# miuda-ai/lele

Hardware: AMD Instinct MI355X
Metric: STFT+mel GB/s (SenseVoice front-end: PCM -> log-mel -> LFR, algorithmic bytes); SenseVoiceSmall-shaped RTF in `sensevoice` (higher is better)
Workload: dtype f32

## Files before the change

lele_amd/csrc/igemm_rs.h:

```cpp
#pragma once

namespace {

struct RsArgs {
    const int8_t* af;
    const int8_t* wf;
    unsigned rows;
    int n;
    int nrt, nct;
    int ncb, nrr;
    int8_t* hid;
    const float* x;
    const float* partial;
    int nblk;
    unsigned* hpart;
    unsigned* sync;
    unsigned* deverr;
#ifdef LELE_HIP_LAB
    long long* dbg;
    int ablate;
#endif
};
#ifdef LELE_HIP_LAB
#define RS_STAMP(who) do { if (g.dbg && lane == 0 && nstamp < 32 && wave < 9) g.dbg[((size_t)blockIdx.x * 9 + wave) * 32 + nstamp++] = (long long)wall_clock64(); } while (0)
// ... 695 lines not shown
        row = row < rows ? row : rows - 1u;
        r.scale = 1.0f;
        r.zp_i = epi.zp_a_fixed;
        if (epi.prm) {
            const unsigned sl = single ? 0u : row / mu;
            r.scale = epi.prm[sl].scale;
            r.zp_i = epi.prm[sl].zp_i;
        }
    };
    auto compute = [&](const v4i (&a)[KW], const Row& r, int t, int buf) {
        const unsigned row = (unsigned)t * 32u + (unsigned)l31;
        const bool rok = row < rows;
        const size_t at = (size_t)(rok ? row : rows - 1u) * (unsigned)n + (unsigned)(cok ? col : n - 4);
        float4 res1, res2;
        if (NRES > 0) res1 = *reinterpret_cast<const float4*>(epi.res1 + at);
        if (NRES > 1) res2 = *reinterpret_cast<const float4*>(epi.res2 + at);
        v16i acc;
#pragma unroll
        for (int i = 0; i < 16; ++i) acc[i] = 0;
        int rsp = 0;
#pragma unroll
        for (int s = 0; s < KW; ++s) {
            acc = __builtin_amdgcn_mfma_i32_32x32x32_i8(bf[s], a[s], acc, 0, 0, 0);
            rsp = __builtin_amdgcn_sdot4(a[s][0], 0x01010101, rsp, false);
            rsp = __builtin_amdgcn_sdot4(a[s][1], 0x01010101, rsp, false);
            rsp = __builtin_amdgcn_sdot4(a[s][2], 0x01010101, rsp, false);
            rsp = __builtin_amdgcn_sdot4(a[s][3], 0x01010101, rsp, false);
        }
#pragma unroll
        for (int gq = 0; gq < 4; ++gq) s_x[buf][wave][gq][lane] = v4i{acc[4 * gq], acc[4 * gq + 1], acc[4 * gq + 2], acc[4 * gq + 3]};
        s_rs[buf][wave][lane] = rsp;
        __syncthreads();
        v4i tot = s_x[buf][0][wave][lane];
        int rowsum = s_rs[buf][0][l31] + s_rs[buf][0][l31 + 32];
#pragma unroll
        for (int w = 1; w < 4; ++w) {
            const v4i p = s_x[buf][w][wave][lane];
            tot[0] += p[0], tot[1] += p[1], tot[2] += p[2], tot[3] += p[3];
            rowsum += s_rs[buf][w][l31] + s_rs[buf][w][l31 + 32];
        }
        const int ca = 128 - r.zp_i;
        const int rterm = cbz * rowsum + epi.k * ca * cbz;
        float4 o;
        o.x = rs_value(tot[0], rterm, ca, colsum[0], r.scale * ws[0], bias[0], has_ws, has_bias, epi.relu);
        o.y = rs_value(tot[1], rterm, ca, colsum[1], r.scale * ws[1], bias[1], has_ws, has_bias, epi.relu);
        o.z = rs_value(tot[2], rterm, ca, colsum[2], r.scale * ws[2], bias[2], has_ws, has_bias, epi.relu);
        o.w = rs_value(tot[3], rterm, ca, colsum[3], r.scale * ws[3], bias[3], has_ws, has_bias, epi.relu);
        if (NRES > 0) o.x = o.x + res1.x, o.y = o.y + res1.y, o.z = o.z + res1.z, o.w = o.w + res1.w;
        if (NRES > 1) o.x = o.x + res2.x, o.y = o.y + res2.y, o.z = o.z + res2.z, o.w = o.w + res2.w;
        if (rok && cok) *reinterpret_cast<float4*>(epi.out + at) = o;
    };
    v4i a0[KW], a1[KW];
    Row r0, r1;
    load_tile(a0, r0, t0);
    int t = t0;
    while (t + 1 < t1) {
        load_tile(a1, r1, t + 1);
        compute(a0, r0, t, 0);
        load_tile(a0, r0, t + 2 < t1 ? t + 2 : t1 - 1);
        compute(a1, r1, t + 1, 1);
        t += 2;
    }
    if (t < t1) compute(a0, r0, t, 0);
}

struct AsArgs {
    const float* x;
    const int8_t* wf;
    unsigned rows;
    int n, nct;
    const float* partial;
    int nblk;
    QParams* prm;
    int tpw;
    const float* ln_g = nullptr;
    const float* ln_b = nullptr;
    float ln_eps = 0.0f;
    float* ln_out = nullptr;
    float* ln_rowstat = nullptr;
    const float* fs_x = nullptr;
    int fs_pitch = 0;
    const float* fs_w = nullptr;
    const float* fs_b = nullptr;
};
constexpr int AS_LN_PITCH = 516;
constexpr int AS_LN_LDS = 32 * AS_LN_PITCH * 4;
constexpr int as_fs_lds(int fs) { return (32 + fs - 1) * AS_LN_PITCH * 4; }

__device__ __forceinline__ void as_ln_rows(const float* s_ln, const float* s_lng, const float* s_lnb, unsigned t, int wave, int hv, int l31,
                                           unsigned rows, float eps, float* ln_out, float* ln_rowstat) {
    constexpr int NT = 16;
    const float inv_n = 1.0f / 512.0f;
#pragma unroll
    for (int rr = 0; rr < 2; ++rr) {
        const int r = 2 * wave + hv + 16 * rr;
        const unsigned grow = t * 32u + (unsigned)r;
        float v[NT];
#pragma unroll
        for (int c = 0; c < NT; ++c) v[c] = s_ln[r * AS_LN_PITCH + 32 * c + l31];
        float sum, sumsq;
        row_sums_reg<NT, true, true>(v, 512, l31, &sum, &sumsq);
        const float mean = sum * inv_n;
        const float var = sumsq * inv_n - mean * mean;
        const float inv_std = 1.0f / sqrtf(var + eps);
        float mn = 3.40282347e+38f, mx = -3.40282347e+38f;
        float* orow = ln_out + (size_t)(grow < rows ? grow : rows - 1u) * 512u;
#pragma unroll
        for (int c = 0; c < NT; ++c) {
            const float tv = (v[c] - mean) * inv_std;
            const float o = fmaf_(tv, s_lng[32 * c + l31], s_lnb[32 * c + l31]);
            if (grow < rows) orow[32 * c + l31] = o;
            mn = o < mn ? o : mn;
            mx = o > mx ? o : mx;
        }
        if (ln_rowstat) {
            mn = group_allreduce32(mn, [](float cur, float a) { return a < cur ? a : cur; });
            mx = group_allreduce32(mx, [](float cur, float a) { return a > cur ? a : cur; });
            if (l31 == 0 && grow < rows) {
                ln_rowstat[2 * (size_t)grow] = mn;
                ln_rowstat[2 * (size_t)grow + 1] = mx;
            }
        }
    }
}

template <int NRES, bool RELU, bool TWO = true, bool LN = false, int FS = 0>
__global__ __launch_bounds__(512) void igemm_as_kernel(AsArgs g, IgemmEpi epi) {
    static_assert(!LN || TWO, "the LayerNorm needs whole rows in one workgroup");
    static_assert(FS == 0 || (LN && NRES >= 1), "the in-kernel FSMN block is res1 of the LayerNorm form");
    constexpr int KS = 16;
    extern __shared__ __attribute__((aligned(16))) float s_ln[];
    __shared__ float s_lng[LN ? 512 : 1], s_lnb[LN ? 512 : 1];
    __shared__ __attribute__((aligned(16))) char s_tile[KS * 1024];
    __shared__ int s_rowsum[4][32];
    __shared__ float s_scale[32];
    __shared__ int s_zp[32];
    __shared__ __attribute__((aligned(16))) int s_colsum[512];
    __shared__ __attribute__((aligned(16))) float s_ws[512];
    __shared__ __attribute__((aligned(16))) float s_bias[512];
    const int lane = threadIdx.x & 63, wave = __builtin_amdgcn_readfirstlane(threadIdx.x >> 6);
    const int hv = lane >> 5, l31 = lane & 31;
    const int t = blockIdx.x, n = g.n;
    const unsigned rows = g.rows, mu = (unsigned)epi.m;
    const int u = wave >> 2, kq = wave & 3, q4 = lane & 3, rsub = lane >> 2;
    const unsigned row_q = (unsigned)t * 32u + 16u * (unsigned)u + (unsigned)rsub;
    const unsigned rowc_q = row_q < rows ? row_q : rows - 1u;
    const unsigned first = (unsigned)t * 32u + 16u * (unsigned)u;
    const unsigned last = first + 15u < rows ? first + 15u : rows - 1u;
    const unsigned s_lo = (first < rows ? first : rows - 1u) / mu, s_hi = last / mu;
    float2 pw[2][4];
#pragma unroll
    for (int a = 0; a < 2; ++a) {
        const unsigned sl = s_lo + (unsigned)a < s_hi ? s_lo + (unsigned)a : s_hi;
        const float2* pp = reinterpret_cast<const float2*>(g.partial) + (size_t)sl * g.nblk;
#pragma unroll
        for (int j = 0; j < 4; ++j) {
            const int idx = lane + 64 * j;
            pw[a][j] = pp[idx < g.nblk ? idx : g.nblk - 1];
        }
    }
    float4 xv[8];
    {
        const float* src = g.x + (size_t)rowc_q * 512u + 128u * (unsigned)kq + 4u * (unsigned)q4;
#pragma unroll
        for (int c = 0; c < 8; ++c) xv[c] = *reinterpret_cast<const float4*>(src + 16 * c);
    }
    float fw[FS > 0 ? FS : 1], fbv = 0.0f;
    if constexpr (FS > 0) {
        const unsigned tile_base = (unsigned)(uintptr_t)(__attribute__((address_space(3))) float*)s_ln;
#pragma unroll
        for (int k2 = 0; k2 < (2 * (32 + FS - 1) + 7) / 8; ++k2) {
            const int it = wave + 8 * k2;
            if (it < 2 * (32 + FS - 1)) {
                const int wr = it >> 1, half = it & 1;
                int gr = (int)t * 32 - FS / 2 + wr;
                gr = gr < 0 ? 0 : (gr < (int)rows ? gr : (int)rows - 1);
                rs_dma16(g.fs_x + (size_t)gr * (unsigned)g.fs_pitch + 256 * half + 4 * lane,
                         __builtin_amdgcn_readfirstlane(tile_base + (unsigned)(wr * AS_LN_PITCH * 4 + 1024 * half)));
            }
        }
#pragma unroll
        for (int j = 0; j < FS; ++j) fw[j] = g.fs_w[threadIdx.x * FS + j];
        fbv = (g.fs_b ? g.fs_b : g.fs_w)[threadIdx.x];
    }
    const int ccol = (int)threadIdx.x < n ? (int)threadIdx.x : n - 1;
    const int csum = epi.col_sums[ccol];
    const float wsv = epi.wscale[epi.wscale_len <= 1 ? 0 : ccol];
    const float bv = (epi.bias ? epi.bias : epi.wscale)[epi.bias ? ccol : 0];
    float lgv = 0.0f, lbv = 0.0f;
    if constexpr (LN) lgv = g.ln_g[threadIdx.x], lbv = g.ln_b[threadIdx.x];
    __builtin_amdgcn_sched_barrier(0);
    const int ct0 = TWO ? 2 * wave : (int)blockIdx.y * g.tpw + wave, ct1 = 2 * wave + 1;
    const bool live0 = (TWO || wave < g.tpw) && ct0 < g.nct;
    v4i bf0[KS], bf1[TWO ? KS : 1];
    {
        const v4i* w0 = reinterpret_cast<const v4i*>(g.wf) + (size_t)(ct0 < g.nct ? ct0 : g.nct - 1) * KS * 64 + lane;
#pragma unroll
        for (int s = 0; s < KS; ++s) bf0[s] = w0[s * 64];
        if constexpr (TWO) {
            const v4i* w1 = reinterpret_cast<const v4i*>(g.wf) + (size_t)(ct1 < g.nct ? ct1 : g.nct - 1) * KS * 64 + lane;
#pragma unroll
            for (int s = 0; s < KS; ++s) bf1[s] = w1[s * 64];
        }
    }
    __builtin_amdgcn_sched_barrier(0);
    s_colsum[threadIdx.x] = csum;
    s_ws[threadIdx.x] = wsv;
    s_bias[threadIdx.x] = epi.bias ? bv : -0.0f;
    if constexpr (LN) s_lng[threadIdx.x] = lgv, s_lnb[threadIdx.x] = lbv;
    QParams q = {1.0f, 0.0f, 1.0f, 0};
    {
        const unsigned mine = rowc_q / mu;
        for (unsigned sl = s_lo; sl <= s_hi; ++sl) {
            float mn = 3.40282347e+38f, mx = -3.40282347e+38f;
            const float2* pp = reinterpret_cast<const float2*>(g.partial) + (size_t)sl * g.nblk;
            int i0 = 0;
            if (sl - s_lo < 2u) {
                const int a = (int)(sl - s_lo);
#pragma unroll
                for (int j = 0; j < 4; ++j) {
                    const float2 w = a == 0 ? pw[0][j] : pw[1][j];
                    mn = w.x < mn ? w.x : mn;
                    mx = w.y > mx ? w.y : mx;
                }
                i0 = 256;
            }
            for (; i0 < g.nblk; i0 += 256) {
                float2 w[4];
#pragma unroll
                for (int j = 0; j < 4; ++j) {
                    const int idx = i0 + lane + 64 * j;
                    w[j] = pp[idx < g.nblk ? idx : g.nblk - 1];
                }
#pragma unroll
                for (int j = 0; j < 4; ++j) {
                    mn = w[j].x < mn ? w[j].x : mn;
                    mx = w[j].y > mx ? w[j].y : mx;
                }
            }
            mn = wave_allreduce64(mn, [](float cur, float a) { return a < cur ? a : cur; });
            mx = wave_allreduce64(mx, [](float cur, float a) { return a > cur ? a : cur; });
            const QParams qs = make_qparams(mn, mx);
            if (mine == sl) q = qs;
            if (kq == 0 && q4 == 0 && row_q < rows && row_q == sl * mu && blockIdx.y == 0) g.prm[sl] = qs;
        }
    }
    {
        unsigned us = 0u;
#pragma unroll
        for (int c = 0; c < 8; ++c) {
            unsigned p = 0u;
            p = __builtin_amdgcn_cvt_pk_u8_f32(__builtin_fmaf(xv[c].x, q.inv_scale, q.zp), 0, p);
            p = __builtin_amdgcn_cvt_pk_u8_f32(__builtin_fmaf(xv[c].y, q.inv_scale, q.zp), 1, p);
            p = __builtin_amdgcn_cvt_pk_u8_f32(__builtin_fmaf(xv[c].z, q.inv_scale, q.zp), 2, p);
            p = __builtin_amdgcn_cvt_pk_u8_f32(__builtin_fmaf(xv[c].w, q.inv_scale, q.zp), 3, p);
            us = __builtin_amdgcn_sad_u8(p, 0u, us);
            *reinterpret_cast<unsigned*>(s_tile + (4 * kq + (c >> 1)) * 1024 + ((16 * u + rsub) + 32 * (c & 1)) * 16 + 4 * q4) = p ^ 0x80808080u;
        }
        us += (unsigned)__shfl_xor((int)us, 1);
        us += (unsigned)__shfl_xor((int)us, 2);
        if (q4 == 0) {
            s_rowsum[kq][16 * u + rsub] = (int)us - 128 * 128;
            if (kq == 0) {
                s_scale[16 * u + rsub] = q.scale;
                s_zp[16 * u + rsub] = q.zp_i;
            }
        }
    }
    __syncthreads();
    if constexpr (FS > 0) {
        const int ch = (int)threadIdx.x;
        constexpr int PL = FS / 2;
        float win[FS];
#pragma unroll
        for (int j = 0; j < FS - 1; ++j) win[j] = s_ln[j * AS_LN_PITCH + ch];
        const int T = (int)mu;
        int tt = (int)(((unsigned)t * 32u) % mu);
#pragma unroll
        for (int r = 0; r < 32; ++r) {
            win[FS - 1] = s_ln[(r + FS - 1) * AS_LN_PITCH + ch];
            float a = 0.0f;
            if (tt >= PL && tt + (FS - 1 - PL) < T) {
#pragma unroll
                for (int j = 0; j < FS; ++j) a = fmaf_(win[j], fw[j], a);
            } else {
#pragma unroll
                for (int j = 0; j < FS; ++j) {
                    const int tq = tt - PL + j;
                    const float f = fmaf_(win[j], fw[j], a);
                    a = (tq >= 0 && tq < T) ? f : a;
                }
            }
            if (g.fs_b) a = a + fbv;
            a = a + win[PL];
            s_ln[r * AS_LN_PITCH + ch] = a;
#pragma unroll
            for (int j = 0; j < FS - 1; ++j) win[j] = win[j + 1];
            tt = tt + 1 == T ? 0 : tt + 1;
        }
        __syncthreads();
    }
    if (!TWO && !live0) return;
    const unsigned row = (unsigned)t * 32u + (unsigned)l31;
    const bool rok = row < rows;
    const unsigned rowc = rok ? row : rows - 1u;
    const float ds = s_scale[l31];
    v16i acc0, acc1;
    {
        const int rowsum = s_rowsum[0][l31] + s_rowsum[1][l31] + s_rowsum[2][l31] + s_rowsum[3][l31];
        const int ca = 128 - s_zp[l31], cbz = 128 - epi.zp_b;
        const int rterm = cbz * rowsum + epi.k * ca * cbz;
#pragma unroll
        for (int gq = 0; gq < 4; ++gq) {
            const v4i c0 = *reinterpret_cast<const v4i*>(&s_colsum[(ct0 * 32 + 4 * hv + 8 * gq) & 511]);
#pragma unroll
            for (int e = 0; e < 4; ++e) acc0[4 * gq + e] = __mul24(ca, c0[e]) + rterm;
            if constexpr (TWO) {
                const v4i c1 = *reinterpret_cast<const v4i*>(&s_colsum[(ct1 * 32 + 4 * hv + 8 * gq) & 511]);
#pragma unroll
                for (int e = 0; e < 4; ++e) acc1[4 * gq + e] = __mul24(ca, c1[e]) + rterm;
            }
        }
    }
    float4 ra1[NRES > 0 ? 4 : 1], ra2[NRES > 1 ? 4 : 1], rb1[NRES > 0 ? 4 : 1], rb2[NRES > 1 ? 4 : 1];
    if (NRES > 0) {
#pragma unroll
        for (int gq = 0; gq < 4; ++gq) {
            const int c0 = ct0 * 32 + 4 * hv + 8 * gq, c1 = ct1 * 32 + 4 * hv + 8 * gq;
            const unsigned at0 = rowc * (unsigned)n + (unsigned)(c0 < n ? c0 : n - 4), at1 = rowc * (unsigned)n + (unsigned)(c1 < n ? c1 : n - 4);
            if constexpr (FS == 0) {
                ra1[gq] = *reinterpret_cast<const float4*>(epi.res1 + at0);
                if (TWO) rb1[gq] = *reinterpret_cast<const float4*>(epi.res1 + at1);
            }
            if (NRES > 1) {
                ra2[gq] = *reinterpret_cast<const float4*>(epi.res2 + at0);
                if (TWO) rb2[gq] = *reinterpret_cast<const float4*>(epi.res2 + at1);
            }
        }
        __builtin_amdgcn_sched_barrier(0);
    }
    {
        const v4i* ap = reinterpret_cast<const v4i*>(s_tile) + lane;
#pragma unroll
        for (int s = 0; s < KS; ++s) {
            const v4i a = ap[s * 64];
            acc0 = __builtin_amdgcn_mfma_i32_32x32x32_i8(bf0[s], a, acc0, 0, 0, 0);
            if constexpr (TWO) acc1 = __builtin_amdgcn_mfma_i32_32x32x32_i8(bf1[s], a, acc1, 0, 0, 0);
        }
    }
    const auto out_rsrc = __builtin_amdgcn_make_buffer_rsrc((void*)epi.out, 0, (int)(rows * (unsigned)n * 4u), 0x00020000);
    auto finish = [&](const v16i& acc, int ct, const float4 (&res1)[NRES > 0 ? 4 : 1], const float4 (&res2)[NRES > 1 ? 4 : 1]) {
        const unsigned obase = rowc * (unsigned)n + (unsigned)(ct * 32 + 4 * hv);
        float smn = 3.40282347e+38f, smx = -3.40282347e+38f;
#pragma unroll
        for (int gq = 0; gq < 4; ++gq) {
            const int cl = (ct * 32 + 4 * hv + 8 * gq) & 511;
            const float4 ws = *reinterpret_cast<const float4*>(&s_ws[cl]);
            const float4 bs = *reinterpret_cast<const float4*>(&s_bias[cl]);
            auto val = [&](int total, float w, float b) {
                float vf = (float)total;
                vf = vf * (ds * w);
                vf = vf + b;
                if (RELU) vf = relu0(vf);
                return vf;
            };
            float4 o;
            o.x = val(acc[4 * gq + 0], ws.x, bs.x);
            o.y = val(acc[4 * gq + 1], ws.y, bs.y);
            o.z = val(acc[4 * gq + 2], ws.z, bs.z);
            o.w = val(acc[4 * gq + 3], ws.w, bs.w);
            if (NRES > 0) {
                float4 r1;
                if constexpr (FS > 0) r1 = *reinterpret_cast<const float4*>(&s_ln[l31 * AS_LN_PITCH + ct * 32 + 4 * hv + 8 * gq]);
                else r1 = res1[gq];
                o.x = o.x + r1.x, o.y = o.y + r1.y, o.z = o.z + r1.z, o.w = o.w + r1.w;
                if (NRES > 1) o.x = o.x + res2[gq].x, o.y = o.y + res2[gq].y, o.z = o.z + res2[gq].z, o.w = o.w + res2[gq].w;
            }
            const bool cok = ct * 32 + 4 * hv + 8 * gq < n;
            const v4u bits = {__float_as_uint(o.x), __float_as_uint(o.y), __float_as_uint(o.z), __float_as_uint(o.w)};
            __builtin_amdgcn_raw_buffer_store_b128(bits, out_rsrc, rok && cok ? (obase + 8u * gq) * 4u : 0xffffffffu, 0, 0);
            if constexpr (LN) *reinterpret_cast<float4*>(&s_ln[l31 * AS_LN_PITCH + ct * 32 + 4 * hv + 8 * gq]) = o;
            if (rok && cok) {
                smn = fminf(smn, fminf(fminf(o.x, o.y), fminf(o.z, o.w)));
                smx = fmaxf(smx, fmaxf(fmaxf(o.x, o.y), fmaxf(o.z, o.w)));
            }
        }
        if (epi.blockstat && ct < g.nct) {
            smn = wave_allreduce64(smn, [](float cur, float x) { return x < cur ? x : cur; });
            smx = wave_allreduce64(smx, [](float cur, float x) { return x > cur ? x : cur; });
            if (lane == 0) {
                float* so = epi.blockstat + ((size_t)t * g.nct + ct) * 2;
                so[0] = smn;
                so[1] = smx;
            }
        }
    };
    finish(acc0, ct0, ra1, ra2);
    if constexpr (TWO) finish(acc1, ct1, rb1, rb2);
    if constexpr (LN) {
        __syncthreads();
        as_ln_rows(s_ln, s_lng, s_lnb, (unsigned)t, wave, hv, l31, rows, g.ln_eps, g.ln_out, g.ln_rowstat);
    }
}

struct AskArgs {
    const int8_t* af;
    const int8_t* wf;
    unsigned rows;
    const float* ln_g = nullptr;
    const float* ln_b = nullptr;
    float ln_eps = 0.0f;
    float* ln_out = nullptr;
    float* ln_rowstat = nullptr;
};
constexpr int ASK_TILE = 64 * 1024;
constexpr int ASK_LDS = ASK_TILE + AS_LN_LDS;
template <int NRES, bool LN>
__global__ __launch_bounds__(512) void igemm_ask_kernel(AskArgs g, IgemmEpi epi) {
    constexpr int KS = 64, RING = 8;
    extern __shared__ __attribute__((aligned(16))) char ask_lds[];
    float* s_ln = reinterpret_cast<float*>(ask_lds + ASK_TILE);
    __shared__ __attribute__((aligned(16))) int s_colsum[512];
    __shared__ __attribute__((aligned(16))) float s_ws[512];
    __shared__ __attribute__((aligned(16))) float s_bias[512];
    __shared__ float s_lng[LN ? 512 : 1], s_lnb[LN ? 512 : 1];
    const int lane = threadIdx.x & 63, wave = __builtin_amdgcn_readfirstlane(threadIdx.x >> 6);
    const int hv = lane >> 5, l31 = lane & 31;
    const unsigned t = blockIdx.x, rows = g.rows, mu = (unsigned)epi.m;
    constexpr int n = 512;
    {
        const unsigned base = (unsigned)(uintptr_t)(__attribute__((address_space(3))) char*)ask_lds;
        const char* src = reinterpret_cast<const char*>(g.af) + ((size_t)t * KS) * 1024 + lane * 16;
#pragma unroll
        for (int j = 0; j < KS / 8; ++j) {
            const int blk = wave + 8 * j;
            rs_dma16(src + (size_t)blk * 1024, __builtin_amdgcn_readfirstlane(base + (unsigned)blk * 1024u));
        }
    }
    const int csum = epi.col_sums[threadIdx.x];
    const float wsv = epi.wscale[epi.wscale_len <= 1 ? 0 : threadIdx.x];
    const float bv = (epi.bias ? epi.bias : epi.wscale)[epi.bias ? threadIdx.x : 0];
    float lgv = 0.0f, lbv = 0.0f;
    if constexpr (LN) lgv = g.ln_g[threadIdx.x], lbv = g.ln_b[threadIdx.x];
    const unsigned row = t * 32u + (unsigned)l31;
    const bool rok = row < rows;
    const unsigned rowc = rok ? row : rows - 1u;
    const unsigned sl = rows == mu ? 0u : rowc / mu;
    const float ds = epi.prm[sl].scale;
    const int zp_i = epi.prm[sl].zp_i;
    __builtin_amdgcn_sched_barrier(0);
    const int ct0 = 2 * wave, ct1 = 2 * wave + 1;
    const v4i* w0 = reinterpret_cast<const v4i*>(g.wf) + (size_t)ct0 * KS * 64 + lane;
    const v4i* w1 = reinterpret_cast<const v4i*>(g.wf) + (size_t)ct1 * KS * 64 + lane;
    const int rot = (int)((blockIdx.x >> 3) & 7u) * 8;
    v4i ra[RING], rb[RING];
#pragma unroll
    for (int s = 0; s < RING; ++s) ra[s] = w0[((s + rot) & (KS - 1)) * 64], rb[s] = w1[((s + rot) & (KS - 1)) * 64];
    __builtin_amdgcn_sched_barrier(0);
    s_colsum[threadIdx.x] = csum;
    s_ws[threadIdx.x] = wsv;
    s_bias[threadIdx.x] = epi.bias ? bv : -0.0f;
    if constexpr (LN) s_lng[threadIdx.x] = lgv, s_lnb[threadIdx.x] = lbv;
    float4 ra1[NRES > 0 ? 4 : 1], ra2[NRES > 1 ? 4 : 1], rb1[NRES > 0 ? 4 : 1], rb2[NRES > 1 ? 4 : 1];
    if (NRES > 0) {
#pragma unroll
        for (int gq = 0; gq < 4; ++gq) {
            const unsigned at0 = rowc * (unsigned)n + (unsigned)(ct0 * 32 + 4 * hv + 8 * gq), at1 = rowc * (unsigned)n + (unsigned)(ct1 * 32 + 4 * hv + 8 * gq);
            ra1[gq] = *reinterpret_cast<const float4*>(epi.res1 + at0);
            rb1[gq] = *reinterpret_cast<const float4*>(epi.res1 + at1);
            if (NRES > 1) {
                ra2[gq] = *reinterpret_cast<const float4*>(epi.res2 + at0);
                rb2[gq] = *reinterpret_cast<const float4*>(epi.res2 + at1);
            }
        }
    }
    __syncthreads();
    v16i acc0, acc1;
#pragma unroll
    for (int i = 0; i < 16; ++i) acc0[i] = 0, acc1[i] = 0;
    int rsp = 0;
    {
        const v4i* ap = reinterpret_cast<const v4i*>(ask_lds) + lane;
#pragma unroll
        for (int s = 0; s < KS; ++s) {
            const v4i a = ap[((s + rot) & (KS - 1)) * 64];
            acc0 = __builtin_amdgcn_mfma_i32_32x32x32_i8(ra[s % RING], a, acc0, 0, 0, 0);
            acc1 = __builtin_amdgcn_mfma_i32_32x32x32_i8(rb[s % RING], a, acc1, 0, 0, 0);
            rsp = __builtin_amdgcn_sdot4(a[0], 0x01010101, rsp, false);
            rsp = __builtin_amdgcn_sdot4(a[1], 0x01010101, rsp, false);
            rsp = __builtin_amdgcn_sdot4(a[2], 0x01010101, rsp, false);
            rsp = __builtin_amdgcn_sdot4(a[3], 0x01010101, rsp, false);
            if (s + RING < KS) ra[s % RING] = w0[((s + RING + rot) & (KS - 1)) * 64], rb[s % RING] = w1[((s + RING + rot) & (KS - 1)) * 64];
        }
    }
    const int rowsum = rsp + __shfl_xor(rsp, 32);
    const int ca = 128 - zp_i, cbz = 128 - epi.zp_b;
    const int rterm = cbz * rowsum + epi.k * ca * cbz;
    const auto out_rsrc = __builtin_amdgcn_make_buffer_rsrc((void*)epi.out, 0, (int)(rows * (unsigned)n * 4u), 0x00020000);
    auto finish = [&](const v16i& acc, int ct, const float4 (&res1)[NRES > 0 ? 4 : 1], const float4 (&res2)[NRES > 1 ? 4 : 1]) {
        const unsigned obase = rowc * (unsigned)n + (unsigned)(ct * 32 + 4 * hv);
#pragma unroll
        for (int gq = 0; gq < 4; ++gq) {
            const int cl = ct * 32 + 4 * hv + 8 * gq;
            const float4 ws = *reinterpret_cast<const float4*>(&s_ws[cl]);
            const float4 bs = *reinterpret_cast<const float4*>(&s_bias[cl]);
            const v4i cs = *reinterpret_cast<const v4i*>(&s_colsum[cl]);
            auto val = [&](int a, int c, float w, float b) {
                float vf = (float)(a + rterm + __mul24(ca, c));
                vf = vf * (ds * w);
                vf = vf + b;
                if (epi.relu) vf = relu0(vf);
                return vf;
            };
            float4 o;
            o.x = val(acc[4 * gq + 0], cs[0], ws.x, bs.x);
            o.y = val(acc[4 * gq + 1], cs[1], ws.y, bs.y);
            o.z = val(acc[4 * gq + 2], cs[2], ws.z, bs.z);
            o.w = val(acc[4 * gq + 3], cs[3], ws.w, bs.w);
            if (NRES > 0) {
                o.x = o.x + res1[gq].x, o.y = o.y + res1[gq].y, o.z = o.z + res1[gq].z, o.w = o.w + res1[gq].w;
                if (NRES > 1) o.x = o.x + res2[gq].x, o.y = o.y + res2[gq].y, o.z = o.z + res2[gq].z, o.w = o.w + res2[gq].w;
            }
            const v4u bits = {__float_as_uint(o.x), __float_as_uint(o.y), __float_as_uint(o.z), __float_as_uint(o.w)};
            __builtin_amdgcn_raw_buffer_store_b128(bits, out_rsrc, rok ? (obase + 8u * gq) * 4u : 0xffffffffu, 0, 0);
            if constexpr (LN) *reinterpret_cast<float4*>(&s_ln[l31 * AS_LN_PITCH + cl]) = o;
        }
    };
    finish(acc0, ct0, ra1, ra2);
    finish(acc1, ct1, rb1, rb2);
    if constexpr (LN) {
        __syncthreads();
        as_ln_rows(s_ln, s_lng, s_lnb, t, wave, hv, l31, rows, g.ln_eps, g.ln_out, g.ln_rowstat);
    }
}

}
```

lele_amd/csrc/quant.hip:

```cpp
#include "common.h"
#include "lane_ops.h"
#include "gemm_small.h"
#include "norm_core.h"

#include <math.h>
#include <stdlib.h>

#include <algorithm>

using namespace lele;

namespace {

typedef int v4i __attribute__((ext_vector_type(4)));
typedef int v16i __attribute__((ext_vector_type(16)));
typedef unsigned v4u __attribute__((ext_vector_type(4)));
typedef float v2f __attribute__((ext_vector_type(2)));

struct QParams {
    float scale, zp, inv_scale;
    int zp_i;
};

__global__ __launch_bounds__(256) void qminmax_kernel(const float* __restrict__ x, int64_t slice_len,
// ... 1310 lines not shown
struct RsFq {
    const float* x = nullptr;
    const float* partial = nullptr;
    int nblk = 0;
    unsigned* hpart = nullptr;
    unsigned* sync = nullptr;
};
unsigned* rs_sync_counters(LeleCtx* ctx, int64_t rows, int64_t n) {
    if (env_int("LELE_HIP_FFN_ONE_LAUNCH", 1) == 0) return nullptr;
    int ncb = 0, nrr = 0;
    rs_grid(ctx, rows, n, &ncb, &nrr);
    const int64_t nrt = (rows + 31) / 32, tiles = (nrt + nrr - 1) / nrr;
    if (tiles > RS_NS_BOTH || nrr > 64 || ncb * nrr > ctx->num_cus || n % 256 != 0) return nullptr;
    if (ctx->lane != 0 || ctx->side_lanes || lele::live_contexts(ctx->device) != 1) return nullptr;
    auto it = ctx->rs_sync.find({ncb, nrr});
    if (it != ctx->rs_sync.end()) return it->second;
    if (ctx->capturing) return nullptr;
    void* p = nullptr;
    const size_t bytes = 256 + (size_t)ncb * nrr * 32;
    if (hipMalloc(&p, bytes) != hipSuccess || hipMemsetAsync(p, 0, bytes, ctx->stream) != hipSuccess) {
        (void)hipGetLastError();
        if (p) (void)hipFree(p);
        return nullptr;
    }
    ctx->rs_sync[{ncb, nrr}] = (unsigned*)p;
    return (unsigned*)p;
}
int launch_rs(LeleCtx* ctx, int em, const int8_t* af, const int8_t* wf, int64_t rows, int n, int8_t* hid, const IgemmEpi& epi,
              const RsFq& fq = RsFq()) {
    const float* x_f32 = fq.x;
    RsArgs g{af, wf, (unsigned)rows, n, (int)((rows + 31) / 32), (n + 31) / 32, 0, 0, hid, x_f32, fq.partial, fq.nblk, fq.hpart};
    g.sync = fq.sync;
    g.deverr = ctx->deverr_dev;
#ifdef LELE_HIP_LAB
    g.dbg = nullptr;
    g.ablate = lab_int("LELE_HIP_RS_ABLATE", 0);
    if (const char* e = lab_env("LELE_HIP_RS_STAMPS"))
        if (lab_int("LELE_HIP_RS_STAMPS_EM", em) == em) g.dbg = (long long*)(uintptr_t)strtoull(e, nullptr, 0);
#endif
    rs_grid(ctx, rows, n, &g.ncb, &g.nrr);
    const dim3 grid((unsigned)(g.ncb * g.nrr));
    const int nres = epi.res1 ? (epi.res2 ? 2 : 1) : 0;
#define LELE_RS(EM_, NRES_, RELU_)                                                                   \
    do {                                                                                             \
        if (x_f32) {                                                                                 \
            auto kern = igemm_rs_kernel<EM_, NRES_, RELU_, true>;                                     \
            LELE_HIP_CHECK(ensure_dyn_lds(reinterpret_cast<const void*>(kern), RS_LDS));              \
            hipLaunchKernelGGL(kern, grid, dim3(768), RS_LDS, ctx->stream, g, epi);                   \
        } else {                                                                                     \
            auto kern = igemm_rs_kernel<EM_, NRES_, RELU_>;                                           \
            LELE_HIP_CHECK(ensure_dyn_lds(reinterpret_cast<const void*>(kern), RS_LDS));              \
            hipLaunchKernelGGL(kern, grid, dim3(640), RS_LDS, ctx->stream, g, epi);                   \
        }                                                                                            \
    } while (0)
    if (em == 3) {
        LELE_REQUIRE(x_f32 && fq.sync && fq.hpart, "launch_rs: the one-launch form needs the quantising loaders and its counters");
        auto kern = igemm_rs_kernel<3, 0, true, true>;
        LELE_HIP_CHECK(ensure_dyn_lds(reinterpret_cast<const void*>(kern), RS_LDS_BOTH));
        hipLaunchKernelGGL(kern, grid, dim3(768), RS_LDS_BOTH, ctx->stream, g, epi);
    } else if (em == 1) LELE_RS(1, 0, true);
    else if (em == 2) LELE_RS(2, 0, true);
    else if (epi.relu) {
        if (nres == 0) LELE_RS(0, 0, true);
        else if (nres == 1) LELE_RS(0, 1, true);
        else LELE_RS(0, 2, true);
    } else {
        if (nres == 0) LELE_RS(0, 0, false);
        else if (nres == 1) LELE_RS(0, 1, false);
        else LELE_RS(0, 2, false);
    }
#undef LELE_RS
    LELE_HIP_CHECK(hipGetLastError());
    return 0;
}
bool as_fits(LeleCtx* ctx, int64_t rows, int64_t n, int64_t k, const void* dx) {
    if (env_int("LELE_HIP_IGEMM_RS", 1) == 0 || lab_int("LELE_HIP_IGEMM_AS", 1) == 0) return false;
    return k == 512 && n <= 512 && n % 4 == 0 && n >= 4 && rows * n < (int64_t(1) << 30) && (((uintptr_t)dx) & 15) == 0 &&
           rows >= (int64_t)lab_int("LELE_HIP_IGEMM_AS_MIN_ROWS", 256);
}
bool as_two(LeleCtx* ctx, int64_t rows, int n) {
    const int64_t nrt = (rows + 31) / 32;
    return nrt * 3 >= (int64_t)ctx->num_cus || (n + 31) / 32 <= 4 || lab_int("LELE_HIP_IGEMM_AS_TPW", 0) == 16;
}
struct AsLn {
    const float* g = nullptr;
    const float* b = nullptr;
    float eps = 0.0f;
    float* out = nullptr;
    float* rowstat = nullptr;
    const float* fs_x = nullptr;
    int fs_pitch = 0;
    const float* fs_w = nullptr;
    const float* fs_b = nullptr;
    int fs_pl = 0;
};
int launch_as(LeleCtx* ctx, const float* x, const int8_t* wf, int64_t rows, int n, const float* partial, int nblk, QParams* prm,
              const IgemmEpi& epi, const AsLn* ln = nullptr) {
    AsArgs g{x, wf, (unsigned)rows, n, (n + 31) / 32, partial, nblk, prm, 16};
    const int64_t nrt = (rows + 31) / 32;
    const bool two = as_two(ctx, rows, n);
    if (!two) g.tpw = lab_int("LELE_HIP_IGEMM_AS_TPW", nrt * 6 >= (int64_t)ctx->num_cus ? 8 : 4);
    const dim3 grid((unsigned)nrt, two ? 1u : (unsigned)((g.nct + g.tpw - 1) / g.tpw));
    const int nres = epi.res1 ? (epi.res2 ? 2 : 1) : 0;
    if (ln) {
        LELE_REQUIRE(two && n == 512 && !epi.relu, "launch_as: the LayerNorm epilogue needs whole 512-wide rows in a workgroup");
        g.ln_g = ln->g, g.ln_b = ln->b, g.ln_eps = ln->eps, g.ln_out = ln->out, g.ln_rowstat = ln->rowstat;
#define LELE_AS_LN(NRES_)                                                                              \
    do {                                                                                               \
        auto kern = igemm_as_kernel<NRES_, false, true, true>;                                          \
        LELE_HIP_CHECK(ensure_dyn_lds(reinterpret_cast<const void*>(kern), AS_LN_LDS));                 \
        hipLaunchKernelGGL(kern, grid, dim3(512), AS_LN_LDS, ctx->stream, g, epi);                      \
    } while (0)
        if (ln->fs_x) {
            g.fs_x = ln->fs_x, g.fs_pitch = ln->fs_pitch, g.fs_w = ln->fs_w, g.fs_b = ln->fs_b;
#define LELE_AS_FS(NRES_)                                                                              \
    do {                                                                                               \
        auto kern = igemm_as_kernel<NRES_, false, true, true, 11>;                                      \
        LELE_HIP_CHECK(ensure_dyn_lds(reinterpret_cast<const void*>(kern), as_fs_lds(11)));             \
        hipLaunchKernelGGL(kern, grid, dim3(512), as_fs_lds(11), ctx->stream, g, epi);                  \
    } while (0)
            if (epi.res2) LELE_AS_FS(2);
            else LELE_AS_FS(1);
#undef LELE_AS_FS
            LELE_HIP_CHECK(hipGetLastError());
            return 0;
        }
        if (nres == 0) LELE_AS_LN(0);
        else if (nres == 1) LELE_AS_LN(1);
        else LELE_AS_LN(2);
#undef LELE_AS_LN
        LELE_HIP_CHECK(hipGetLastError());
        return 0;
    }
#define LELE_AS(NRES_, RELU_)                                                                                     \
    do {                                                                                                          \
        if (two) hipLaunchKernelGGL((igemm_as_kernel<NRES_, RELU_, true>), grid, dim3(512), 0, ctx->stream, g, epi);   \
        else hipLaunchKernelGGL((igemm_as_kernel<NRES_, RELU_, false>), grid, dim3(512), 0, ctx->stream, g, epi);     \
    } while (0)
    if (epi.relu) {
        if (nres == 0) LELE_AS(0, true);
        else if (nres == 1) LELE_AS(1, true);
        else LELE_AS(2, true);
    } else {
        if (nres == 0) LELE_AS(0, false);
        else if (nres == 1) LELE_AS(1, false);
        else LELE_AS(2, false);
    }
#undef LELE_AS
    LELE_HIP_CHECK(hipGetLastError());
    return 0;
}
int launch_rs_ks4(LeleCtx* ctx, const int8_t* af, const int8_t* wf, int64_t rows, int n, const IgemmEpi& epi) {
    RsArgs g{af, wf, (unsigned)rows, n, (int)((rows + 31) / 32), (n + 31) / 32, 0, 0, nullptr};
#ifdef LELE_HIP_LAB
    g.dbg = nullptr;
    g.ablate = 0;
#endif
    g.nrr = std::max(1, std::min(g.nrt, 2 * ctx->num_cus / g.nct));
    const dim3 grid((unsigned)(g.nct * g.nrr));
    const int nres = epi.res1 ? (epi.res2 ? 2 : 1) : 0;
    if (nres == 0) hipLaunchKernelGGL(igemm_rs_ks4_kernel<0>, grid, dim3(256), 0, ctx->stream, g, epi);
    else if (nres == 1) hipLaunchKernelGGL(igemm_rs_ks4_kernel<1>, grid, dim3(256), 0, ctx->stream, g, epi);
    else hipLaunchKernelGGL(igemm_rs_ks4_kernel<2>, grid, dim3(256), 0, ctx->stream, g, epi);
    LELE_HIP_CHECK(hipGetLastError());
    return 0;
}

bool ask_fits(LeleCtx* ctx, int64_t rows, int64_t n, int64_t k) {
    return env_int("LELE_HIP_IGEMM_RS", 1) != 0 && env_int("LELE_HIP_IGEMM_ASK", 1) != 0 && k == 2048 && n == 512 && rows * n < (int64_t(1) << 30) &&
           as_two(ctx, rows, (int)n);
}
int launch_ask(LeleCtx* ctx, const int8_t* af, const int8_t* wf, int64_t rows, const IgemmEpi& epi, const AsLn* ln) {
    AskArgs g{af, wf, (unsigned)rows};
    if (ln) g.ln_g = ln->g, g.ln_b = ln->b, g.ln_eps = ln->eps, g.ln_out = ln->out, g.ln_rowstat = ln->rowstat;
    const dim3 grid((unsigned)((rows + 31) / 32));
    const int nres = epi.res1 ? (epi.res2 ? 2 : 1) : 0;
#define LELE_ASK(NRES_, LN_)                                                                            \
    do {                                                                                                \
        auto kern = igemm_ask_kernel<NRES_, LN_>;                                                        \
        LELE_HIP_CHECK(ensure_dyn_lds(reinterpret_cast<const void*>(kern), (LN_) ? ASK_LDS : ASK_TILE)); \
        hipLaunchKernelGGL(kern, grid, dim3(512), (LN_) ? ASK_LDS : ASK_TILE, ctx->stream, g, epi);      \
    } while (0)
    if (ln) {
        if (nres == 0) LELE_ASK(0, true);
        else if (nres == 1) LELE_ASK(1, true);
        else LELE_ASK(2, true);
    } else {
#ifdef LELE_HIP_LAB
        if (nres == 0) LELE_ASK(0, false);
        else if (nres == 1) LELE_ASK(1, false);
        else LELE_ASK(2, false);
#else
        LELE_REQUIRE(false, "launch_ask: the form without a LayerNorm is built into the lab library only");
#endif
    }
#undef LELE_ASK
    LELE_HIP_CHECK(hipGetLastError());
    return 0;
}

}

namespace lele {
int quant_params_of(LeleCtx* ctx, const float* const* srcs, const int64_t* lens, int nsrc, void* prm_dev) {
    int64_t total_blocks = 0;
    std::vector<int> nb(nsrc);
    for (int i = 0; i < nsrc; ++i) {
        nb[i] = (int)std::max<int64_t>(1, std::min<int64_t>(256, (lens[i] + 4095) / 4096));
        total_blocks += nb[i];
    }
    void* partial = nullptr;
    LELE_TRY(ctx->arena_alloc((size_t)total_blocks * 8, &partial));
    int64_t off = 0;
    for (int i = 0; i < nsrc; ++i) {
        if (lens[i] > 0)
            hipLaunchKernelGGL(qminmax_kernel, dim3(nb[i], 1), dim3(256), 0, ctx->stream, srcs[i], lens[i],
                               (float*)partial + 2 * off);
        else
            nb[i] = 0;
        off += nb[i];
    }
    hipLaunchKernelGGL(qparams_kernel, dim3(1), dim3(64), 0, ctx->stream, (const float*)partial, (int)off, (QParams*)prm_dev,
                       (float*)nullptr, (float*)nullptr);
    LELE_HIP_CHECK(hipGetLastError());
    return 0;
}
}

namespace {
void find_partials(LeleCtx* ctx, const LeleTensor* input, int64_t batch, int64_t m, int64_t k, const float** partial, int* nblk) {
    const int64_t rows = batch * m;
    *partial = nullptr;
    *nblk = 0;
    if (input->mem != LELE_MEM_DEVICE || m > 2048) return;
    auto it = ctx->buf_of_data.find(input->data);
    if (it == ctx->buf_of_data.end() || !it->second->rowstat_valid) return;
    const LeleBuf* src = it->second;
    if (src->rowstat_kind == 0 && src->rowstat_len == k && src->rowstat_rows == rows) {
        *partial = src->rowstat;
        *nblk = (int)m;
    } else if (src->rowstat_kind == 2 && src->rowstat_len == k && src->rowstat_m == m && src->rowstat_batch == batch && src->rowstat_rows % batch == 0) {
        *partial = src->rowstat;
        *nblk = (int)(src->rowstat_rows / batch);
    } else if (src->rowstat_kind == 1 && batch == 1 && src->rowstat_len == rows * k && src->rowstat_rows <= 4096) {
        *partial = src->rowstat;
        *nblk = (int)src->rowstat_rows;
    }
}

int first_scalar_of(LeleCtx* ctx, const LeleTensor* t, float* v) {
    *v = 0.0f;
    if (!t || numel(t) == 0) return 0;
    if (t->mem != LELE_MEM_DEVICE) {
        *v = *(const float*)t->data;
        return 0;
    }
    LELE_HIP_CHECK(hipMemcpyAsync(v, t->data, 4, hipMemcpyDeviceToHost, ctx->stream));
    LELE_REQUIRE(!ctx->capturing, "graph capture: this op must run once eagerly first (it allocates or synchronises)");
// ... 888 lines not shown
```

Before: 1859.

## Size igemm AS workgroups by rows-per-CU to spread small row counts

Adds a rows-per-workgroup parameter to the int8 AS and ASK GEMM kernels so that, for the two-tile form, each workgroup can take fewer than 32 rows (at least 8) and the grid covers more CUs when the row count is small. Row bounds, the FSMN window, the LayerNorm epilogue and the ASK activation addressing are rewritten in terms of the per-workgroup row range, and the FSMN input rows are prefetched eight at a time. It also adds lab-only timestamp instrumentation. The cost is MFMA tiles that are partly idle when a workgroup holds fewer than 32 rows.

```diff
diff --git a/lele_amd/csrc/igemm_rs.h b/lele_amd/csrc/igemm_rs.h
--- a/lele_amd/csrc/igemm_rs.h
+++ b/lele_amd/csrc/igemm_rs.h
@@ -801,19 +801,25 @@
     int fs_pitch = 0;
     const float* fs_w = nullptr;
     const float* fs_b = nullptr;
+    unsigned rpw = 32;
+#ifdef LELE_HIP_LAB
+    long long* dbg = nullptr;
+#endif
 };
 constexpr int AS_LN_PITCH = 516;
 constexpr int AS_LN_LDS = 32 * AS_LN_PITCH * 4;
 constexpr int as_fs_lds(int fs) { return (32 + fs - 1) * AS_LN_PITCH * 4; }
 
-__device__ __forceinline__ void as_ln_rows(const float* s_ln, const float* s_lng, const float* s_lnb, unsigned t, int wave, int hv, int l31,
-                                           unsigned rows, float eps, float* ln_out, float* ln_rowstat) {
+__device__ __forceinline__ void as_ln_rows(const float* s_ln, const float* s_lng, const float* s_lnb, unsigned t, unsigned R, int wave, int hv,
+                                           int l31, unsigned rows, float eps, float* ln_out, float* ln_rowstat) {
     constexpr int NT = 16;
     const float inv_n = 1.0f / 512.0f;
 #pragma unroll
     for (int rr = 0; rr < 2; ++rr) {
+        if ((unsigned)(2 * wave + 16 * rr) >= R) break;
         const int r = 2 * wave + hv + 16 * rr;
-        const unsigned grow = t * 32u + (unsigned)r;
+        const unsigned grow = t * R + (unsigned)r;
+        const bool live = (unsigned)r < R && grow < rows;
         float v[NT];
 #pragma unroll
         for (int c = 0; c < NT; ++c) v[c] = s_ln[r * AS_LN_PITCH + 32 * c + l31];
@@ -823,19 +829,19 @@
         const float var = sumsq * inv_n - mean * mean;
         const float inv_std = 1.0f / sqrtf(var + eps);
         float mn = 3.40282347e+38f, mx = -3.40282347e+38f;
-        float* orow = ln_out + (size_t)(grow < rows ? grow : rows - 1u) * 512u;
+        float* orow = ln_out + (size_t)(live ? grow : rows - 1u) * 512u;
 #pragma unroll
         for (int c = 0; c < NT; ++c) {
             const float tv = (v[c] - mean) * inv_std;
             const float o = fmaf_(tv, s_lng[32 * c + l31], s_lnb[32 * c + l31]);
-            if (grow < rows) orow[32 * c + l31] = o;
+            if (live) orow[32 * c + l31] = o;
             mn = o < mn ? o : mn;
             mx = o > mx ? o : mx;
         }
         if (ln_rowstat) {
             mn = group_allreduce32(mn, [](float cur, float a) { return a < cur ? a : cur; });
             mx = group_allreduce32(mx, [](float cur, float a) { return a > cur ? a : cur; });
-            if (l31 == 0 && grow < rows) {
+            if (l31 == 0 && live) {
                 ln_rowstat[2 * (size_t)grow] = mn;
                 ln_rowstat[2 * (size_t)grow + 1] = mx;
             }
@@ -861,12 +867,17 @@
     const int hv = lane >> 5, l31 = lane & 31;
     const int t = blockIdx.x, n = g.n;
     const unsigned rows = g.rows, mu = (unsigned)epi.m;
+    const unsigned R = TWO ? g.rpw : 32u;
+    const unsigned wg_first = (unsigned)t * R;
+    const unsigned wg_last = wg_first + R - 1u < rows ? wg_first + R - 1u : rows - 1u;
     const int u = wave >> 2, kq = wave & 3, q4 = lane & 3, rsub = lane >> 2;
-    const unsigned row_q = (unsigned)t * 32u + 16u * (unsigned)u + (unsigned)rsub;
-    const unsigned rowc_q = row_q < rows ? row_q : rows - 1u;
-    const unsigned first = (unsigned)t * 32u + 16u * (unsigned)u;
-    const unsigned last = first + 15u < rows ? first + 15u : rows - 1u;
-    const unsigned s_lo = (first < rows ? first : rows - 1u) / mu, s_hi = last / mu;
+    const unsigned row_q = wg_first + 16u * (unsigned)u + (unsigned)rsub;
+    const unsigned rowc_q = row_q < wg_last ? row_q : wg_last;
+    const unsigned first = wg_first + 16u * (unsigned)u;
+    const unsigned last = first + 15u < wg_last ? first + 15u : wg_last;
+    const unsigned s_lo = (first < wg_last ? first : wg_last) / mu, s_hi = last / mu;
+    int nstamp = 0;
+    RS_STAMP(0);
     float2 pw[2][4];
 #pragma unroll
     for (int a = 0; a < 2; ++a) {
@@ -890,9 +901,9 @@
 #pragma unroll
         for (int k2 = 0; k2 < (2 * (32 + FS - 1) + 7) / 8; ++k2) {
             const int it = wave + 8 * k2;
-            if (it < 2 * (32 + FS - 1)) {
+            if (it < 2 * ((int)R + FS - 1)) {
                 const int wr = it >> 1, half = it & 1;
-                int gr = (int)t * 32 - FS / 2 + wr;
+                int gr = (int)wg_first - FS / 2 + wr;
                 gr = gr < 0 ? 0 : (gr < (int)rows ? gr : (int)rows - 1);
                 rs_dma16(g.fs_x + (size_t)gr * (unsigned)g.fs_pitch + 256 * half + 4 * lane,
                          __builtin_amdgcn_readfirstlane(tile_base + (unsigned)(wr * AS_LN_PITCH * 4 + 1024 * half)));
@@ -961,7 +972,7 @@
             mx = wave_allreduce64(mx, [](float cur, float a) { return a > cur ? a : cur; });
             const QParams qs = make_qparams(mn, mx);
             if (mine == sl) q = qs;
-            if (kq == 0 && q4 == 0 && row_q < rows && row_q == sl * mu && blockIdx.y == 0) g.prm[sl] = qs;
+            if (kq == 0 && q4 == 0 && row_q <= wg_last && row_q == sl * mu && blockIdx.y == 0) g.prm[sl] = qs;
         }
     }
     {
@@ -986,18 +997,25 @@
             }
         }
     }
+    RS_STAMP(0);
     __syncthreads();
+    RS_STAMP(0);
     if constexpr (FS > 0) {
         const int ch = (int)threadIdx.x;
         constexpr int PL = FS / 2;
-        float win[FS];
+        float win[FS], nxt[8];
 #pragma unroll
         for (int j = 0; j < FS - 1; ++j) win[j] = s_ln[j * AS_LN_PITCH + ch];
         const int T = (int)mu;
-        int tt = (int)(((unsigned)t * 32u) % mu);
+        int tt = (int)(wg_first % mu);
 #pragma unroll
         for (int r = 0; r < 32; ++r) {
-            win[FS - 1] = s_ln[(r + FS - 1) * AS_LN_PITCH + ch];
+            if (r % 8 == 0 && (unsigned)r >= R) break;
+            if (r % 8 == 0) {
+#pragma unroll
+                for (int i = 0; i < 8; ++i) nxt[i] = s_ln[(r + i + FS - 1) * AS_LN_PITCH + ch];
+            }
+            win[FS - 1] = nxt[r % 8];
             float a = 0.0f;
             if (tt >= PL && tt + (FS - 1 - PL) < T) {
 #pragma unroll
@@ -1018,11 +1036,12 @@
             tt = tt + 1 == T ? 0 : tt + 1;
         }
         __syncthreads();
+        RS_STAMP(0);
     }
     if (!TWO && !live0) return;
-    const unsigned row = (unsigned)t * 32u + (unsigned)l31;
-    const bool rok = row < rows;
-    const unsigned rowc = rok ? row : rows - 1u;
+    const unsigned row = wg_first + (unsigned)l31;
+    const bool rok = row <= wg_last;
+    const unsigned rowc = rok ? row : wg_last;
     const float ds = s_scale[l31];
     v16i acc0, acc1;
     {
@@ -1067,6 +1086,7 @@
             if constexpr (TWO) acc1 = __builtin_amdgcn_mfma_i32_32x32x32_i8(bf1[s], a, acc1, 0, 0, 0);
         }
     }
+    RS_STAMP(0);
     const auto out_rsrc = __builtin_amdgcn_make_buffer_rsrc((void*)epi.out, 0, (int)(rows * (unsigned)n * 4u), 0x00020000);
     auto finish = [&](const v16i& acc, int ct, const float4 (&res1)[NRES > 0 ? 4 : 1], const float4 (&res2)[NRES > 1 ? 4 : 1]) {
         const unsigned obase = rowc * (unsigned)n + (unsigned)(ct * 32 + 4 * hv);
@@ -1116,9 +1136,12 @@
     };
     finish(acc0, ct0, ra1, ra2);
     if constexpr (TWO) finish(acc1, ct1, rb1, rb2);
+    RS_STAMP(0);
     if constexpr (LN) {
         __syncthreads();
-        as_ln_rows(s_ln, s_lng, s_lnb, (unsigned)t, wave, hv, l31, rows, g.ln_eps, g.ln_out, g.ln_rowstat);
+        RS_STAMP(0);
+        as_ln_rows(s_ln, s_lng, s_lnb, (unsigned)t, R, wave, hv, l31, rows, g.ln_eps, g.ln_out, g.ln_rowstat);
+        RS_STAMP(0);
     }
 }
 
@@ -1131,6 +1154,10 @@
     float ln_eps = 0.0f;
     float* ln_out = nullptr;
     float* ln_rowstat = nullptr;
+    unsigned rpw = 32;
+#ifdef LELE_HIP_LAB
+    long long* dbg = nullptr;
+#endif
 };
 constexpr int ASK_TILE = 64 * 1024;
 constexpr int ASK_LDS = ASK_TILE + AS_LN_LDS;
@@ -1147,9 +1174,14 @@
     const int hv = lane >> 5, l31 = lane & 31;
     const unsigned t = blockIdx.x, rows = g.rows, mu = (unsigned)epi.m;
     constexpr int n = 512;
+    const unsigned R = g.rpw, wg_first = t * R;
+    const unsigned wg_last = wg_first + R - 1u < rows ? wg_first + R - 1u : rows - 1u;
+    int nstamp = 0;
+    RS_STAMP(0);
     {
         const unsigned base = (unsigned)(uintptr_t)(__attribute__((address_space(3))) char*)ask_lds;
-        const char* src = reinterpret_cast<const char*>(g.af) + ((size_t)t * KS) * 1024 + lane * 16;
+        const unsigned grow = wg_first + (unsigned)l31 < wg_last ? wg_first + (unsigned)l31 : wg_last;
+        const char* src = reinterpret_cast<const char*>(g.af) + ((size_t)(grow >> 5) * KS) * 1024 + ((grow & 31u) + 32u * (unsigned)hv) * 16;
 #pragma unroll
         for (int j = 0; j < KS / 8; ++j) {
             const int blk = wave + 8 * j;
@@ -1161,9 +1193,9 @@
     const float bv = (epi.bias ? epi.bias : epi.wscale)[epi.bias ? threadIdx.x : 0];
     float lgv = 0.0f, lbv = 0.0f;
     if constexpr (LN) lgv = g.ln_g[threadIdx.x], lbv = g.ln_b[threadIdx.x];
-    const unsigned row = t * 32u + (unsigned)l31;
-    const bool rok = row < rows;
-    const unsigned rowc = rok ? row : rows - 1u;
+    const unsigned row = wg_first + (unsigned)l31;
+    const bool rok = row <= wg_last;
+    const unsigned rowc = rok ? row : wg_last;
     const unsigned sl = rows == mu ? 0u : rowc / mu;
     const float ds = epi.prm[sl].scale;
     const int zp_i = epi.prm[sl].zp_i;
@@ -1193,7 +1225,9 @@
             }
         }
     }
+    RS_STAMP(0);
     __syncthreads();
+    RS_STAMP(0);
     v16i acc0, acc1;
 #pragma unroll
     for (int i = 0; i < 16; ++i) acc0[i] = 0, acc1[i] = 0;
@@ -1210,6 +1244,7 @@
             rsp = __builtin_amdgcn_sdot4(a[2], 0x01010101, rsp, false);
             rsp = __builtin_amdgcn_sdot4(a[3], 0x01010101, rsp, false);
             if (s + RING < KS) ra[s % RING] = w0[((s + RING + rot) & (KS - 1)) * 64], rb[s % RING] = w1[((s + RING + rot) & (KS - 1)) * 64];
+            if (s % 16 == 15) RS_STAMP(0);
         }
     }
     const int rowsum = rsp + __shfl_xor(rsp, 32);
@@ -1247,9 +1282,12 @@
     };
     finish(acc0, ct0, ra1, ra2);
     finish(acc1, ct1, rb1, rb2);
+    RS_STAMP(0);
     if constexpr (LN) {
         __syncthreads();
-        as_ln_rows(s_ln, s_lng, s_lnb, t, wave, hv, l31, rows, g.ln_eps, g.ln_out, g.ln_rowstat);
+        RS_STAMP(0);
+        as_ln_rows(s_ln, s_lng, s_lnb, t, R, wave, hv, l31, rows, g.ln_eps, g.ln_out, g.ln_rowstat);
+        RS_STAMP(0);
     }
 }
 
diff --git a/lele_amd/csrc/quant.hip b/lele_amd/csrc/quant.hip
--- a/lele_amd/csrc/quant.hip
+++ b/lele_amd/csrc/quant.hip
@@ -1416,6 +1416,20 @@
     const int64_t nrt = (rows + 31) / 32;
     return nrt * 3 >= (int64_t)ctx->num_cus || (n + 31) / 32 <= 4 || lab_int("LELE_HIP_IGEMM_AS_TPW", 0) == 16;
 }
+constexpr int AS_RPW_MIN = 8;
+int as_rows_per_wg(LeleCtx* ctx, int64_t rows, bool deal_rows, unsigned* rpw) {
+    const int forced = env_int("LELE_HIP_IGEMM_ROWS_PER_WG", 0);
+    LELE_REQUIRE(forced == 0 || (forced >= AS_RPW_MIN && forced <= 32), "LELE_HIP_IGEMM_ROWS_PER_WG: 0 (automatic) or 8 .. 32");
+    const int64_t even = (rows + ctx->num_cus - 1) / ctx->num_cus;
+    *rpw = forced ? (unsigned)forced : deal_rows ? (unsigned)std::min<int64_t>(32, std::max<int64_t>(AS_RPW_MIN, even)) : 32u;
+    return 0;
+}
+#ifdef LELE_HIP_LAB
+long long* as_stamps(int em) {
+    const char* e = lab_env("LELE_HIP_RS_STAMPS");
+    return e && lab_int("LELE_HIP_RS_STAMPS_EM", -1) == em ? (long long*)(uintptr_t)strtoull(e, nullptr, 0) : nullptr;
+}
+#endif
 struct AsLn {
     const float* g = nullptr;
     const float* b = nullptr;
@@ -1434,7 +1448,11 @@
     const int64_t nrt = (rows + 31) / 32;
     const bool two = as_two(ctx, rows, n);
     if (!two) g.tpw = lab_int("LELE_HIP_IGEMM_AS_TPW", nrt * 6 >= (int64_t)ctx->num_cus ? 8 : 4);
-    const dim3 grid((unsigned)nrt, two ? 1u : (unsigned)((g.nct + g.tpw - 1) / g.tpw));
+    if (two && !epi.blockstat) LELE_TRY(as_rows_per_wg(ctx, rows, true, &g.rpw));
+#ifdef LELE_HIP_LAB
+    if (two) g.dbg = as_stamps(10);
+#endif
+    const dim3 grid(two ? (unsigned)((rows + g.rpw - 1) / g.rpw) : (unsigned)nrt, two ? 1u : (unsigned)((g.nct + g.tpw - 1) / g.tpw));
     const int nres = epi.res1 ? (epi.res2 ? 2 : 1) : 0;
     if (ln) {
         LELE_REQUIRE(two && n == 512 && !epi.relu, "launch_as: the LayerNorm epilogue needs whole 512-wide rows in a workgroup");
@@ -1507,7 +1525,11 @@
 int launch_ask(LeleCtx* ctx, const int8_t* af, const int8_t* wf, int64_t rows, const IgemmEpi& epi, const AsLn* ln) {
     AskArgs g{af, wf, (unsigned)rows};
     if (ln) g.ln_g = ln->g, g.ln_b = ln->b, g.ln_eps = ln->eps, g.ln_out = ln->out, g.ln_rowstat = ln->rowstat;
-    const dim3 grid((unsigned)((rows + 31) / 32));
+    LELE_TRY(as_rows_per_wg(ctx, rows, false, &g.rpw));
+#ifdef LELE_HIP_LAB
+    g.dbg = as_stamps(11);
+#endif
+    const dim3 grid((unsigned)((rows + g.rpw - 1) / g.rpw));
     const int nres = epi.res1 ? (epi.res2 ? 2 : 1) : 0;
 #define LELE_ASK(NRES_, LN_)                                                                            \
     do {                                                                                                \
```

New measurement: 1850. Within noise of the previous version (-0.5%).
